# gongaa/Feedback-GNN

Measured on AMD Instinct MI355X. Metric: decoded codewords/sec, [[882,24]] 64-iter BP4 + feedback-GNN, higher is better.
Workload: dtype f32

## Files before the change

### feedback_gnn_amd/_lib.py

```python
import ctypes as C
import os
import subprocess

_HERE = os.path.dirname(os.path.abspath(__file__))
LIB_PATH = os.path.join(_HERE, "lib", "libfgnn_hip.so")
CSRC = os.path.join(_HERE, "csrc")

CN_TYPES = {"boxplus": 0, "boxplus-phi": 1, "minsum": 2}
ROWS_X_LOGIT, ROWS_Z_LOGIT, ROWS_HX_PERP, ROWS_HZ_PERP, ROWS_LX, ROWS_LZ = 0, 1, 2, 3, 4, 5


class FgnnError(RuntimeError):
    pass


def build(force=False, verbose=False):
    cmd = ["make", "-C", CSRC, "-j4"] + (["-B"] if force else [])
    res = subprocess.run(cmd, stdout=subprocess.PIPE, stderr=subprocess.STDOUT, text=True)
    if verbose or res.returncode != 0:
        print(res.stdout)
    if res.returncode != 0:
        raise FgnnError("building libfgnn_hip.so failed")
    return LIB_PATH


KERNEL_SOURCES = {
    "bp4": ("fgnn_bp4.hip", "fgnn_math.h", "fgnn_internal.h", "fgnn_rng.h", "fgnn_cn.h", "Makefile"),
    "gnn": ("fgnn_gnn.hip", "fgnn_math.h", "fgnn_internal.h", "fgnn_pk.h", "fgnn_mlp.h", "Makefile"),
    "gnnbp4": ("fgnn_gnnbp4.hip", "fgnn_math.h", "fgnn_internal.h", "fgnn_pk.h", "fgnn_mlp.h", "Makefile"),
}


def source_fingerprint(kind):
    import hashlib
    h = hashlib.sha256()
    for name in KERNEL_SOURCES[kind]:
        h.update(name.encode() + b"\0")
        with open(os.path.join(CSRC, name), "rb") as f:
            h.update(f.read())
        h.update(b"\0")
    return h.hexdigest()


def library_sha256(path=None):
    import hashlib
    h = hashlib.sha256()
    with open(path or os.environ.get("FGNN_LIB_PATH", LIB_PATH), "rb") as f:
        for blk in iter(lambda: f.read(1 << 20), b""):
            h.update(blk)
    return h.hexdigest()


_SIGNATURES = {
    "fgnn_last_error": (C.c_char_p, []),
    "fgnn_version": (C.c_int, []),
    "fgnn_graph_create": (C.c_int, [C.c_int, C.c_int, C.c_int, C.c_int, C.c_void_p, C.c_void_p, C.c_int, C.c_void_p,
                                    C.c_void_p, C.c_int, C.POINTER(C.c_void_p)]),
    "fgnn_graph_destroy": (None, [C.c_void_p]),
    "fgnn_graph_set_rows": (C.c_int, [C.c_void_p, C.c_int, C.c_int, C.c_int, C.c_void_p, C.c_void_p]),
    "fgnn_graph_set_launch": (C.c_int, [C.c_void_p, C.c_int, C.c_int]),
    "fgnn_graph_set_option": (C.c_int, [C.c_void_p, C.c_int, C.c_int]),
    "fgnn_graph_force_generic": (C.c_int, [C.c_void_p, C.c_int]),
    "fgnn_graph_info": (C.c_int, [C.c_void_p, C.c_void_p]),
    "fgnn_graph_edges": (C.c_int, [C.c_void_p, C.c_int, C.c_void_p, C.c_void_p]),
    "fgnn_profile_enable": (C.c_int, [C.c_void_p, C.c_int]),
    "fgnn_profile_read": (C.c_int, [C.c_void_p, C.c_void_p, C.c_void_p, C.c_void_p, C.c_int, C.c_void_p]),
    "fgnn_bp4_decode": (C.c_int, [C.c_void_p, C.c_int, C.c_int, C.c_float, C.c_void_p, C.c_float, C.c_void_p, C.c_void_p,
                                  C.c_int] + [C.c_void_p] * 10),
    "fgnn_bp4_decode_trace": (C.c_int, [C.c_void_p, C.c_int, C.c_int, C.c_float, C.c_void_p, C.c_float, C.c_void_p, C.c_void_p,
                                        C.c_int] + [C.c_void_p] * 10),
    "fgnn_weights_create": (C.c_int, [C.c_void_p, C.c_int, C.POINTER(C.c_void_p)]),
    "fgnn_weights_destroy": (None, [C.c_void_p]),
    "fgnn_feedback_gnn": (C.c_int, [C.c_void_p] * 7 + [C.c_int, C.c_void_p, C.c_void_p]),
    "fgnn_pauli_noise": (C.c_int, [C.c_uint64, C.c_float, C.c_uint64, C.c_int, C.c_int, C.c_void_p, C.c_void_p, C.c_void_p]),
    "fgnn_pauli_noise_xyz": (C.c_int, [C.c_uint64, C.c_float, C.c_float, C.c_float, C.c_uint64, C.c_int, C.c_int, C.c_void_p, C.c_void_p, C.c_void_p]),
    "fgnn_pauli_noise_wt": (C.c_int, [C.c_uint64, C.c_int, C.c_uint64, C.c_int, C.c_int, C.c_void_p, C.c_void_p, C.c_void_p]),
    "fgnn_pauli_noise_dev": (C.c_int, [C.c_uint64, C.c_float, C.c_void_p, C.c_uint64, C.c_int, C.c_int, C.c_void_p, C.c_void_p, C.c_void_p]),
    "fgnn_syndrome": (C.c_int, [C.c_void_p, C.c_void_p, C.c_void_p, C.c_int, C.c_void_p, C.c_void_p, C.c_void_p]),
    "fgnn_flag_update": (C.c_int, [C.c_void_p] * 5 + [C.c_int, C.c_void_p, C.c_void_p]),
    "fgnn_merge": (C.c_int, [C.c_void_p] * 3 + [C.c_int, C.c_int, C.c_void_p, C.c_void_p, C.c_void_p]),
# ... 82 lines not shown
```

### feedback_gnn_amd/csrc/fgnn_bp4.hip

```cpp

#include "fgnn_internal.h"
#include "fgnn_math.h"
#include "fgnn_cn.h"

#ifndef FGNN_BP4_WAVES
#define FGNN_BP4_WAVES 7
#endif
#ifndef FGNN_HWT_PIN_CLIP_POINTS
#define FGNN_HWT_PIN_CLIP_POINTS 1
#endif
#ifndef FGNN_PHI_STAGE
#define FGNN_PHI_STAGE 1
#endif

namespace {

struct BpArgs {
    int B, num_iter, tpc, cpb, lds_per_cw, lch_off;
    float factor, llr_const;
    const float* llr_ch;
    const uint8_t* synd_x;
    const uint8_t* synd_z;
    const float* msg_init_x;
    const float* msg_init_z;
    float* llr_out;
    uint8_t* x_hat;
    uint8_t* z_hat;
    float* x_logit;
    float* z_logit;
    float* msg_out_x;
    float* msg_out_z;
    const int* index;
    int shortcut;
    int early_exit;
    int sig_off;
    int lreg;
    int hwt;
    uint8_t* flagged;
    int flag_off;
    float* gmem;
    float* trace_x;
    float* trace_z;
    int trace_off;
    float* tape_x;
    float* tape_z;
    int shared_lse;
};

template <bool HWT>
struct Mx {
    static __device__ __forceinline__ float softplus(float t) { return fg_softplus(t); }
    static __device__ __forceinline__ float lse2(float a, float b) { return fg_lse2(a, b); }
    static __device__ __forceinline__ float lse2_corr(float a, float b) { return fg_lse2_corr(a, b); }
    static __device__ __forceinline__ float phi(float x) { return fg_phi(x); }
};
template <>
struct Mx<true> {
    static __device__ __forceinline__ float exp(float x) { return __builtin_amdgcn_exp2f(x * FG_LOG2E); }
    static __device__ __forceinline__ float log(float x) { return __builtin_amdgcn_logf(x) * 0.693147182f; }
    static __device__ __forceinline__ float softplus(float t)
    {
        const float y = exp(FG_CLAMP(t, -87.0f, FG_SOFTPLUS_THRESH));
        const float r = (t < -FG_SOFTPLUS_THRESH) ? ((t < -87.0f) ? 0.0f : y) : log(1.0f + y);
        return (t > FG_SOFTPLUS_THRESH) ? t : r;
    }
    static __device__ __forceinline__ float lse2_corr(float a, float b)
    {
        const float y = exp(-FG_MIN(FG_ABS(a - b), 20.0f));
        return log(1.0f + y);
    }
    static __device__ __forceinline__ float lse2(float a, float b)
    {
        return lse2_corr(a, b) + FG_MAX(a, b);
    }
    static __device__ __forceinline__ float phi(float x)
    {
        const float xc = FG_CLAMP(x, FG_PHI_MIN, FG_PHI_MAX);
        const float y = exp(xc);
        const float sp = (xc > FG_SOFTPLUS_THRESH) ? xc : log(1.0f + y);
        float r = sp - log(y - 1.0f);
#if FGNN_HWT_PIN_CLIP_POINTS
        r = (x >= FG_PHI_MAX) ? 0.0f : r;
        r = (x <= FG_PHI_MIN) ? 16.6355324f : r;
#endif
        return r;
    }
};

template <bool HWT = false>
__device__ __forceinline__ float logit_row_opt(const float* llr, const int* __restrict__ col, int deg, float phi0, bool shortcut)
{
    if (shortcut) {
        unsigned neg = 0;
        bool sat = true;
        for (int j = 0; j < deg; ++j) {
            const float v = llr[col[j]];
            neg ^= (v < 0.0f);
            sat = sat && (FG_ABS(v) >= FG_PHI_MAX);
        }
        if (__all(sat)) return with_sign(phi0, neg);
    }
    return logit_row<Mx<HWT>>(llr, col, deg);
}

template <int N, bool HWT = false>
__device__ __forceinline__ void phi_n(const float (&x)[N], float (&out)[N])
{
    if constexpr (HWT) {
#pragma unroll
        for (int k = 0; k < N; ++k) out[k] = Mx<true>::phi(x[k]);
        return;
    }
    const float* tab = fg_log_tab();
    float xc[N], y[N];
    uint32_t eb1[N], eb2[N], j1[N], j2[N];
#pragma unroll
    for (int k = 0; k < N; ++k) {
        xc[k] = FG_CLAMP(x[k], FG_PHI_MIN, FG_PHI_MAX);
        y[k] = fg_exp(xc[k]);
        const uint32_t w1 = fg_f2u(1.0f + y[k]) - FG_LOG_OFFS;
        const uint32_t w2 = fg_f2u(y[k] - 1.0f) - FG_LOG_OFFS;
        eb1[k] = w1 & 0xff800000u;
        eb2[k] = w2 & 0xff800000u;
        j1[k] = (w1 >> 18) & 31u;
        j2[k] = (w2 >> 18) & 31u;
    }
    __builtin_amdgcn_sched_barrier(0);
    float rc1[N], lc1[N], rc2[N], lc2[N];
#pragma unroll
    for (int k = 0; k < N; ++k) {
        rc1[k] = tab[j1[k]];
        lc1[k] = tab[32 + j1[k]];
        rc2[k] = tab[j2[k]];
        lc2[k] = tab[32 + j2[k]];
    }
    __builtin_amdgcn_sched_barrier(0);
#pragma unroll
    for (int k = 0; k < N; ++k) {
        const float a = fg_u2f(fg_f2u(rc1[k]) - eb1[k]);
        const float r1 = FG_FMA(y[k], a, a - 1.0f);
        float sp = FG_FMA((float)(int32_t)eb1[k], FG_LN2_S23, lc1[k] + fg_log1p_small(r1));
        sp = (xc[k] > FG_SOFTPLUS_THRESH) ? xc[k] : sp;
        const float mm = fg_u2f(fg_f2u(y[k] - 1.0f) - eb2[k]);
        const float r2 = FG_FMA(mm, rc2[k], -1.0f);
        const float lg = FG_FMA((float)(int32_t)eb2[k], FG_LN2_S23, lc2[k] + fg_log1p_small(r2));
        out[k] = sp - lg;
    }
}

template <int DC, bool HWT = false, bool F1 = false>
__device__ __forceinline__ bool cn_phi_regular(float* msg, const int (&sl)[DC], unsigned synd, float factor, float phi0,
                                               bool shortcut)
{
    constexpr int H = (DC % FGNN_PHI_STAGE == 0) ? FGNN_PHI_STAGE : DC / 2;
    static_assert(DC % H == 0, "a phi stage must take a whole fraction of a check");
    float v[DC], aa[DC];
    uint32_t neg = synd << 31;
    bool sat = true;
#pragma unroll
    for (int j = 0; j < DC; ++j) {
        v[j] = slot_ref(msg, sl[j]);
        neg ^= fg_f2u(v[j]);
        sat = sat && (FG_ABS(v[j]) >= FG_PHI_MAX);
    }
    if (shortcut && __all(sat)) {
#pragma unroll
        for (int j = 0; j < DC; ++j) {
            const float o = fg_u2f(fg_f2u(phi0) | ((neg ^ fg_f2u(v[j])) & 0x80000000u));
            slot_ref(msg, sl[j]) = F1 ? o : o * factor;
        }
        return true;
    }
#pragma unroll
    for (int g0 = 0; g0 < DC; g0 += H) {
        float xa[H], oa[H];
#pragma unroll
        for (int j = 0; j < H; ++j) xa[j] = FG_ABS(v[g0 + j]);
        phi_n<H, HWT>(xa, oa);
#pragma unroll
        for (int j = 0; j < H; ++j) aa[g0 + j] = oa[j];
    }
    float T = 0.0f;
#pragma unroll
    for (int j = 0; j < DC; ++j) T = T + aa[j];
#pragma unroll
    for (int g0 = 0; g0 < DC; g0 += H) {
        float xa[H], oa[H];
#pragma unroll
        for (int j = 0; j < H; ++j) xa[j] = T - aa[g0 + j];
        phi_n<H, HWT>(xa, oa);
#pragma unroll
        for (int j = 0; j < H; ++j) {
            const float o = fg_u2f(fg_f2u(oa[j]) | ((neg ^ fg_f2u(v[g0 + j])) & 0x80000000u));
            slot_ref(msg, sl[g0 + j]) = F1 ? o : o * factor;
        }
    }
    return false;
}

template <int DC>
__device__ __forceinline__ void cn_tanh_regular(float* msg, const int (&sl)[DC], unsigned synd, float factor)
{
    float t[DC];
    float P = 1.0f;
#pragma unroll
    for (int j = 0; j < DC; ++j) {
        float tj = fg_tanh(slot_ref(msg, sl[j]) / 2.0f);
        tj = (tj == 0.0f) ? 1e-12f : tj;
        P = (j == 0) ? tj : P * tj;
        t[j] = tj;
    }
    P = P * (synd ? -1.0f : 1.0f);
    const float clipv = 0.99999988f;
#pragma unroll
    for (int j = 0; j < DC; ++j) {
        float q = fg_rcp_unit(t[j]) * P;
        q = (FG_ABS(q) < 1e-7f) ? 0.0f : q;
        q = FG_MIN(FG_MAX(q, -clipv), clipv);
        slot_ref(msg, sl[j]) = (2.0f * fg_atanh(q)) * factor;
    }
}

template <bool HWT = false>
__device__ __forceinline__ bool cn_phi_generic(float* msg, const int* __restrict__ slot, int deg, unsigned synd, float factor,
                                               float phi0, bool shortcut)
{
    if (shortcut) {
        unsigned neg = synd;
        bool sat = true;
        for (int j = 0; j < deg; ++j) {
            const float v = msg[slot[j]];
            neg ^= (v < 0.0f);
            sat = sat && (FG_ABS(v) >= FG_PHI_MAX);
        }
        if (__all(sat)) {
            for (int j = 0; j < deg; ++j) {
                const int s = slot[j];
                msg[s] = with_sign(phi0, neg ^ (unsigned)(msg[s] < 0.0f)) * factor;
            }
            return true;
        }
    }
    cn_update<FGNN_CN_BOXPLUS_PHI, Mx<HWT>>(msg, slot, deg, synd, factor);
    return false;
}

__device__ __forceinline__ float softplus_saturated(float t)
{
    const float y = fg_exp(FG_MIN(FG_MAX(t, -87.0f), 0.0f));
    return (t > 0.0f) ? t : ((t < -87.0f) ? 0.0f : y);
}

template <int CN_TYPE, int DVX, int DVZ, int DC, bool OPT, bool HWT = false, int NQ = 0, bool TRACE = false, bool GMEM = false, int LSE = 2>
__global__ void __launch_bounds__(1024) __attribute__((amdgpu_waves_per_eu(NQ > 0 ? FGNN_BP4_WAVES - 1 : FGNN_BP4_WAVES)))
bp4_kernel(GraphDev g, BpArgs a)
{
    static_assert(!(HWT && OPT), "the hardware-transcendental variant is the fixed dataflow only: the exact shortcuts are proofs about fgnn_math.h");
    static_assert(!GMEM || (DVX == 0 && !OPT && !HWT && NQ == 0 && !TRACE), "the global-memory variant is the plain runtime-degree kernel");
    using MX = Mx<HWT>;
    FG_LOG_TAB_SETUP();
    constexpr bool REGULAR = DVX > 0;
    constexpr bool LREG = NQ > 0;
    constexpr int NQA = LREG ? NQ : 1;
    const bool opt_shortcut = OPT && a.shortcut != 0;
    const bool opt_exit = OPT && a.early_exit != 0;
    const bool shl = LSE == 2 ? a.shared_lse != 0 : LSE == 1;
    extern __shared__ float lds[];
    const int cwl = threadIdx.x / a.tpc;
    const int lane = threadIdx.x - cwl * a.tpc;
    const int slot_b = blockIdx.x * a.cpb + cwl;
    const bool active = slot_b < a.B;
    const int b = (active && a.index) ? a.index[slot_b] : slot_b;
    float* msg;
    if constexpr (GMEM) msg = a.gmem + (size_t)slot_b * a.lds_per_cw;
    else msg = lds + (size_t)cwl * a.lds_per_cw;
    float* Lch = msg + a.lch_off;
    const int n = g.n;

    constexpr bool CLOSED_OK = REGULAR && CN_TYPE == FGNN_CN_BOXPLUS_PHI && !LREG && !TRACE;
    const bool zero_start = REGULAR && !TRACE && !a.msg_init_x && !a.msg_init_z && a.num_iter > 0;
    const bool first_closed = CLOSED_OK && zero_start && !a.llr_ch;
    const bool first_peeled = zero_start && a.llr_ch != nullptr;
    const bool fill = !first_closed && !first_peeled;
    if (active) {
        if (fill) {
            for (int e = lane; e < g.E_x; e += a.tpc) msg[e] = a.msg_init_x ? a.msg_init_x[(size_t)b * g.E_x + e] : 0.0f;
            for (int e = lane; e < g.E_z; e += a.tpc)
                msg[g.E_x + e] = a.msg_init_z ? a.msg_init_z[(size_t)b * g.E_z + e] : 0.0f;
        }
        if (a.llr_ch && !LREG)
            for (int i = lane; i < 3 * n; i += a.tpc) Lch[i] = a.llr_ch[(size_t)b * 3 * n + i];
    }
    float lreg[3][NQA];
    if constexpr (LREG) {
#pragma unroll
        for (int i = 0; i < NQ; ++i) {
            const int v = lane + i * a.tpc;
            const bool in = active && v < n;
#pragma unroll
            for (int c = 0; c < 3; ++c) lreg[c][i] = in ? a.llr_ch[(size_t)b * 3 * n + c * n + v] : 0.0f;
        }
    }
    if (fill || (a.llr_ch && !LREG)) __syncthreads();

    const uint8_t* sx = a.synd_x + (size_t)b * g.m_x;
    const uint8_t* sz = a.synd_z + (size_t)b * g.m_z;
    const int lane_c = lane + (a.tpc >> 1) < a.tpc ? lane + (a.tpc >> 1) : lane - a.tpc + (a.tpc >> 1);

    const float phi0 = MX::phi(0.0f);
    (void)phi0;
    unsigned* sigw = reinterpret_cast<unsigned*>(msg + a.sig_off);
    int* flags = reinterpret_cast<int*>(sigw + n);
    bool a1 = false, a2 = false;
    if (opt_exit) {
        for (int v = lane; v < n; v += a.tpc) sigw[v] = fill ? 0xffffffffu : 0u;
        if (lane < 4) flags[lane] = 0;
        __syncthreads();
    }
    int it_begin = 0;
    if constexpr (CLOSED_OK) {
        if (first_closed) {
            const float L = a.llr_const;
            const float Y = (0.0f + 0.0f) + L, X = 0.0f + L, Z = 0.0f + L;
            const float nu_x = MX::softplus(-X) - MX::lse2(-(Z - 0.0f), -(Y - 0.0f));
            const float nu_z = MX::softplus(-Z) - MX::lse2(-(X - 0.0f), -(Y - 0.0f));
            if (active)
                for (int c = lane_c; c < g.m; c += a.tpc) {
                    const unsigned synd = (c < g.m_x ? sx[c] : sz[c - g.m_x]) & 1u;
                    const uint4 pk = reinterpret_cast<const uint4*>(g.cslot16)[c];
                    const unsigned w[4] = {pk.x, pk.y, pk.z, pk.w};
                    const float nu = c < g.m_x ? nu_x : nu_z;
                    const unsigned ng = nu < 0.0f;
                    unsigned neg = synd;
                    const float aa = MX::phi(FG_ABS(nu));
                    float T = 0.0f;
#pragma unroll
                    for (int j = 0; j < DC; ++j) {
                        neg ^= ng;
                        T = T + aa;
                    }
                    const float val = with_sign(MX::phi(T - aa), neg ^ ng) * a.factor;
#pragma unroll
                    for (int j = 0; j < DC; ++j) slot_ref(msg, (int)((w[j >> 1] >> ((j & 1) * 16)) & 0xffffu)) = val;
                }
            if (opt_exit) a1 = FG_ABS(nu_x) >= FG_PHI_MAX && FG_ABS(nu_z) >= FG_PHI_MAX;
            it_begin = 1;
            __syncthreads();
        }
    }
    const bool cn_one = a.cpb == 1, cn_f1 = a.factor == 1.0f;
    unsigned synd_bits = 0;
    if (active) {
        int i = 0;
        for (int c = lane_c; c < g.m && i < 32; c += a.tpc, ++i) synd_bits |= ((c < g.m_x ? sx[c] : sz[c - g.m_x]) & 1u) << i;
    }
    const bool synd_in_reg = (g.m + a.tpc - 1) / a.tpc <= 32;
    auto trace_step = [&](const int k) __attribute__((always_inline)) {
        float* tlx = msg + a.trace_off;
        float* tlz = tlx + n;
        if (active && a.tape_x) {
            float* px = a.tape_x + ((size_t)k * a.B + b) * g.E_x;
            float* pz = a.tape_z + ((size_t)k * a.B + b) * g.E_z;
            for (int e = lane; e < g.E_x; e += a.tpc) px[e] = msg[e];
            for (int e = lane; e < g.E_z; e += a.tpc) pz[e] = msg[g.E_x + e];
        }
        if (active)
            for (int v = lane; v < n; v += a.tpc) {
                const int x0 = g.vptr_x[v], x1 = g.vptr_x[v + 1], z0 = g.vptr_z[v], z1 = g.vptr_z[v + 1];
                float Sz = 0.0f, Sx = 0.0f;
                for (int e = z0; e < z1; ++e) Sz = Sz + msg[e];
                for (int e = x0; e < x1; ++e) Sx = Sx + msg[e];
                const float lx = a.llr_ch ? Lch[v] : a.llr_const, ly = a.llr_ch ? Lch[n + v] : a.llr_const,
                            lz = a.llr_ch ? Lch[2 * n + v] : a.llr_const;
                const float Y = (Sz + Sx) + ly;
                const float X = Sz + lx;
                const float Z = Sx + lz;
                tlz[v] = MX::softplus(-X) - MX::lse2(-Z, -Y);
                tlx[v] = MX::softplus(-Z) - MX::lse2(-X, -Y);
            }
        __syncthreads();
        if (active) {
            float* tx = a.trace_x + ((size_t)k * a.B + b) * g.rows[0];
            for (int r = lane; r < g.rows[0]; r += a.tpc) {
                const int p0 = g.rptr[0][r];
                tx[r] = logit_row<Mx<HWT>>(tlx, g.rcol[0] + p0, g.rptr[0][r + 1] - p0);
            }
            float* tz = a.trace_z + ((size_t)k * a.B + b) * g.rows[1];
            for (int r = lane; r < g.rows[1]; r += a.tpc) {
                const int p0 = g.rptr[1][r];
                tz[r] = logit_row<Mx<HWT>>(tlz, g.rcol[1] + p0, g.rptr[1][r + 1] - p0);
            }
        }
    };
    if constexpr (TRACE) trace_step(0);
    if constexpr (REGULAR && !TRACE) {
        if (first_peeled && active) {
            auto vn_first = [&](const int v, const float lx, const float ly, const float lz) __attribute__((always_inline)) {
                const float Y = (0.0f + 0.0f) + ly;
                const float X = 0.0f + lx;
                const float Z = 0.0f + lz;
                const float numx = MX::softplus(-X);
                const float numz = MX::softplus(-Z);
                const float Ze = Z - 0.0f, Xe = X - 0.0f, Ye = Y - 0.0f;
                float ox, oz;
                if (shl) {
                    ox = numx - (MX::lse2_corr(-Z, -Y) + FG_MAX(-Ze, -Ye));
                    oz = numz - (MX::lse2_corr(-X, -Y) + FG_MAX(-Xe, -Ye));
                } else {
                    ox = numx - MX::lse2(-Ze, -Ye);
                    oz = numz - MX::lse2(-Xe, -Ye);
                }
                float* px = msg + v * DVX;
                float* pz = msg + g.E_x + v * DVZ;
#pragma unroll
                for (int k = 0; k < DVX; ++k) px[k] = ox;
#pragma unroll
                for (int k = 0; k < DVZ; ++k) pz[k] = oz;
            };
            if constexpr (LREG) {
#pragma unroll
                for (int i = 0; i < NQ; ++i) {
                    const int v = lane + i * a.tpc;
                    if (v < n) vn_first(v, lreg[0][i], lreg[1][i], lreg[2][i]);
                }
            } else {
                for (int v = lane; v < n; v += a.tpc) vn_first(v, Lch[v], Lch[n + v], Lch[2 * n + v]);
            }
        }
    }
    for (int it = it_begin; it < a.num_iter; ++it) {
        bool changed = false, cn_slow = false;
        auto vn_body = [&](const int v, const float lx, const float ly, const float lz) __attribute__((always_inline)) {
                if constexpr (REGULAR) {
                    float* px = msg + v * DVX;
                    float* pz = msg + g.E_x + v * DVZ;
                    float mx[DVX], mz[DVZ];
                    float Sz = 0.0f, Sx = 0.0f;
#pragma unroll
                    for (int k = 0; k < DVZ; ++k) { mz[k] = pz[k]; Sz = Sz + mz[k]; }
#pragma unroll
                    for (int k = 0; k < DVX; ++k) { mx[k] = px[k]; Sx = Sx + mx[k]; }
                    if (opt_exit) {
                        unsigned sig = 0;
#pragma unroll
                        for (int k = 0; k < DVX; ++k) sig |= sign_bit(mx[k]) << k;
#pragma unroll
                        for (int k = 0; k < DVZ; ++k) sig |= sign_bit(mz[k]) << (DVX + k);
                        if (sigw[v] != sig) {
                            changed = true;
                            sigw[v] = sig;
                        }
                    }
                    const float Y = (Sz + Sx) + ly;
                    const float X = Sz + lx;
                    const float Z = Sx + lz;
                    bool sat = opt_shortcut && FG_ABS(X) > FG_SOFTPLUS_THRESH && FG_ABS(Z) > FG_SOFTPLUS_THRESH;
                    if (shl) {
                        sat = sat && FG_ABS((-Z) - (-Y)) >= 20.0f && FG_ABS((-X) - (-Y)) >= 20.0f;
                    } else {
#pragma unroll
                        for (int k = 0; k < DVX; ++k) sat = sat && (FG_ABS((Z - mx[k]) - (Y - mx[k])) >= 20.0f);
#pragma unroll
                        for (int k = 0; k < DVZ; ++k) sat = sat && (FG_ABS((X - mz[k]) - (Y - mz[k])) >= 20.0f);
                    }
                    if (opt_shortcut && __all(sat)) {
                        const float numx = softplus_saturated(-X);
                        const float numz = softplus_saturated(-Z);
#pragma unroll
                        for (int k = 0; k < DVX; ++k) {
                            const float Ze = Z - mx[k], Ye = Y - mx[k];
                            px[k] = numx - (0.0f + FG_MAX(-Ze, -Ye));
                        }
#pragma unroll
                        for (int k = 0; k < DVZ; ++k) {
                            const float Xe = X - mz[k], Ye = Y - mz[k];
                            pz[k] = numz - (0.0f + FG_MAX(-Xe, -Ye));
                        }
                        return;
                    }
// ... 46 lines not shown
                            sig |= sign_bit(mm) << ((x1 - x0) + (e - z0));
                        }
                        if (opt_exit && sigw[v] != sig) {
                            changed = true;
                            sigw[v] = sig;
                        }
                        if (__all(sat)) {
                            const float nx = softplus_saturated(-X), nz = softplus_saturated(-Z);
                            for (int e = x0; e < x1; ++e) {
                                const float mm = msg[e];
                                const float Ze = Z - mm, Ye = Y - mm;
                                msg[e] = nx - (0.0f + FG_MAX(-Ze, -Ye));
                            }
                            for (int e = z0; e < z1; ++e) {
                                const float mm = msg[e];
                                const float Xe = X - mm, Ye = Y - mm;
                                msg[e] = nz - (0.0f + FG_MAX(-Xe, -Ye));
                            }
                            return;
                        }
                    }
                    const float numx = MX::softplus(-X);
                    const float numz = MX::softplus(-Z);
                    if (shl) {
                        const float cx = MX::lse2_corr(-Z, -Y), cz = MX::lse2_corr(-X, -Y);
                        for (int e = x0; e < x1; ++e) {
                            float m = msg[e];
                            float Ze = Z - m, Ye = Y - m;
                            msg[e] = numx - (cx + FG_MAX(-Ze, -Ye));
                        }
                        for (int e = z0; e < z1; ++e) {
                            float m = msg[e];
                            float Xe = X - m, Ye = Y - m;
                            msg[e] = numz - (cz + FG_MAX(-Xe, -Ye));
                        }
                        return;
                    }
                    for (int e = x0; e < x1; ++e) {
                        float m = msg[e];
                        float Ze = Z - m, Ye = Y - m;
                        msg[e] = numx - MX::lse2(-Ze, -Ye);
                    }
                    for (int e = z0; e < z1; ++e) {
                        float m = msg[e];
                        float Xe = X - m, Ye = Y - m;
                        msg[e] = numz - MX::lse2(-Xe, -Ye);
                    }
                }
            };
        if (active && !(first_peeled && it == 0)) {
            if constexpr (LREG) {
#pragma unroll
                for (int i = 0; i < NQ; ++i) {
                    const int v = lane + i * a.tpc;
                    if (v < n) vn_body(v, lreg[0][i], lreg[1][i], lreg[2][i]);
                }
            } else {
                for (int v = lane; v < n; v += a.tpc) {
                    if (a.llr_ch) vn_body(v, Lch[v], Lch[n + v], Lch[2 * n + v]);
                    else vn_body(v, a.llr_const, a.llr_const, a.llr_const);
                }
            }
        }
        if (opt_exit && changed) flags[2 * (it & 1)] = 1;
        __syncthreads();
        if (opt_exit && lane == 0) {
            flags[2 * ((it + 1) & 1)] = 0;
            flags[2 * ((it + 1) & 1) + 1] = 0;
        }
        if (active) {
            int ci = 0;
            for (int c = lane_c; c < g.m; c += a.tpc, ++ci) {
                const unsigned synd = synd_in_reg ? (synd_bits >> ci) & 1u : (c < g.m_x ? sx[c] : sz[c - g.m_x]) & 1u;
                if constexpr (REGULAR) {
                    const uint4 pk = reinterpret_cast<const uint4*>(g.cslot16)[c];
                    const unsigned w[4] = {pk.x, pk.y, pk.z, pk.w};
                    int sl[DC];
#pragma unroll
                    for (int j = 0; j < DC; ++j) sl[j] = (int)((w[j >> 1] >> ((j & 1) * 16)) & 0xffffu);
                    if constexpr (CN_TYPE == FGNN_CN_BOXPLUS_PHI) {
                        bool fast;
                        if (cn_one && cn_f1) fast = cn_phi_regular<DC, HWT, true>(lds, sl, synd, 1.0f, phi0, opt_shortcut);
                        else if (cn_one) fast = cn_phi_regular<DC, HWT, false>(lds, sl, synd, a.factor, phi0, opt_shortcut);
                        else fast = cn_phi_regular<DC, HWT, false>(msg, sl, synd, a.factor, phi0, opt_shortcut);
                        cn_slow = !fast || cn_slow;
                    } else if constexpr (CN_TYPE == FGNN_CN_MINSUM) {
                        cn_minsum_regular<DC>(msg, sl, DC, synd, a.factor);
                    } else {
                        cn_tanh_regular<DC>(msg, sl, synd, a.factor);
                    }
                } else {
                    const int c0 = g.cptr[c], deg = g.cptr[c + 1] - c0;
                    if constexpr (CN_TYPE == FGNN_CN_BOXPLUS_PHI)
                        cn_slow = !cn_phi_generic<HWT>(msg, g.cslot + c0, deg, synd, a.factor, phi0, opt_shortcut) || cn_slow;
                    else cn_update<CN_TYPE, Mx<HWT>>(msg, g.cslot + c0, deg, synd, a.factor);
                }
            }
        }
        if (opt_exit && cn_slow) flags[2 * (it & 1) + 1] = 1;
        __syncthreads();
        if (opt_exit) {
            const bool stable = a1 && a2 && flags[2 * (it & 1)] == 0;
            a2 = a1;
            a1 = flags[2 * (it & 1) + 1] == 0;
            if (stable) break;
        }
        if constexpr (TRACE) trace_step(it + 1);
    }

    if (active) {
        if (a.msg_out_x)
            for (int e = lane; e < g.E_x; e += a.tpc) a.msg_out_x[(size_t)b * g.E_x + e] = msg[e];
        if (a.msg_out_z)
            for (int e = lane; e < g.E_z; e += a.tpc) a.msg_out_z[(size_t)b * g.E_z + e] = msg[g.E_x + e];
    }
    auto total_body = [&](const int v, const float lx, const float ly, const float lz) __attribute__((always_inline)) {
            const int x0 = g.vptr_x[v], x1 = g.vptr_x[v + 1], z0 = g.vptr_z[v], z1 = g.vptr_z[v + 1];
            float Sz = 0.0f, Sx = 0.0f;
            for (int e = z0; e < z1; ++e) Sz = Sz + msg[e];
            for (int e = x0; e < x1; ++e) Sx = Sx + msg[e];
            const float Y = (Sz + Sx) + ly;
            const float X = Sz + lx;
            const float Z = Sx + lz;
            float* o = a.llr_out + (size_t)b * 3 * n;
            o[v] = X;
            o[n + v] = Y;
            o[2 * n + v] = Z;
            int d = 0;
            float best = 0.0f;
            if (X < best) { best = X; d = 1; }
            if (Z < best) { best = Z; d = 2; }
            if (Y < best) { best = Y; d = 3; }
            a.x_hat[(size_t)b * n + v] = (uint8_t)(d & 1);
            a.z_hat[(size_t)b * n + v] = (uint8_t)(d >> 1);
    };
    if (active) {
        if constexpr (LREG) {
#pragma unroll
            for (int i = 0; i < NQ; ++i) {
                const int v = lane + i * a.tpc;
                if (v < n) total_body(v, lreg[0][i], lreg[1][i], lreg[2][i]);
            }
        } else {
            for (int v = lane; v < n; v += a.tpc) {
                if (a.llr_ch) total_body(v, Lch[v], Lch[n + v], Lch[2 * n + v]);
                else total_body(v, a.llr_const, a.llr_const, a.llr_const);
            }
        }
    }
    if (a.flagged) {
        uint8_t* dec = reinterpret_cast<uint8_t*>(msg + a.flag_off);
        unsigned* fword = reinterpret_cast<unsigned*>(dec + ((n + 3) & ~3));
        __syncthreads();
        if (active)
            for (int v = lane; v < n; v += a.tpc) {
                dec[v] = (uint8_t)(a.x_hat[(size_t)b * n + v] | (a.z_hat[(size_t)b * n + v] << 1));
            }
        if (lane == 0) *fword = 0u;
        __syncthreads();
        unsigned mine = 0;
        if (active)
            for (int c = lane; c < g.m; c += a.tpc) {
                const int sh = c < g.m_x ? 1 : 0;
                unsigned par = (c < g.m_x ? sx[c] : sz[c - g.m_x]) & 1u;
                for (int e = g.cptr[c]; e < g.cptr[c + 1]; ++e) par ^= (dec[g.cvn[e]] >> sh) & 1u;
                mine |= par;
            }
        if (mine) atomicOr(fword, 1u);
        __syncthreads();
        if (active && lane == 0) a.flagged[b] = (uint8_t)(*fword != 0u);
    }
    if (!a.x_logit && !a.z_logit) return;
    __syncthreads();
    float* llx = msg;
    float* llz = msg + n;
    if (active)
        for (int v = lane; v < n; v += a.tpc) {
            const float* o = a.llr_out + (size_t)b * 3 * n;
            const float X = o[v], Y = o[n + v], Z = o[2 * n + v];
            const bool sat = opt_shortcut && FG_ABS(X) > FG_SOFTPLUS_THRESH && FG_ABS(Z) > FG_SOFTPLUS_THRESH &&
                             FG_ABS((-Z) - (-Y)) >= 20.0f && FG_ABS((-X) - (-Y)) >= 20.0f;
            if (opt_shortcut && __all(sat)) {
                llz[v] = softplus_saturated(-X) - (0.0f + FG_MAX(-Z, -Y));
                llx[v] = softplus_saturated(-Z) - (0.0f + FG_MAX(-X, -Y));
                continue;
            }
            llz[v] = MX::softplus(-X) - MX::lse2(-Z, -Y);
            llx[v] = MX::softplus(-Z) - MX::lse2(-X, -Y);
        }
    __syncthreads();
    if (active) {
        if (a.x_logit)
            for (int r = lane; r < g.rows[0]; r += a.tpc) {
                const int p0 = g.rptr[0][r];
                a.x_logit[(size_t)b * g.rows[0] + r] = logit_row_opt<HWT>(llx, g.rcol[0] + p0, g.rptr[0][r + 1] - p0, phi0, opt_shortcut);
            }
        if (a.z_logit)
            for (int r = lane; r < g.rows[1]; r += a.tpc) {
                const int p0 = g.rptr[1][r];
                a.z_logit[(size_t)b * g.rows[1] + r] = logit_row_opt<HWT>(llz, g.rcol[1] + p0, g.rptr[1][r + 1] - p0, phi0, opt_shortcut);
            }
    }
}

using Bp4Kernel = void (*)(GraphDev, BpArgs);

template <int NQ, bool OPT, int LSE>
constexpr Bp4Kernel bp4_lse_kernel = bp4_kernel<FGNN_CN_BOXPLUS_PHI, 3, 3, 6, OPT, false, NQ, false, false, LSE>;
constexpr Bp4Kernel bp4_lse_kernels[3][2][2] = {
    {{bp4_lse_kernel<0, false, 0>, bp4_lse_kernel<0, false, 1>}, {bp4_lse_kernel<0, true, 0>, bp4_lse_kernel<0, true, 1>}},
    {{bp4_lse_kernel<4, false, 0>, bp4_lse_kernel<4, false, 1>}, {bp4_lse_kernel<4, true, 0>, bp4_lse_kernel<4, true, 1>}},
    {{bp4_lse_kernel<5, false, 0>, bp4_lse_kernel<5, false, 1>}, {bp4_lse_kernel<5, true, 0>, bp4_lse_kernel<5, true, 1>}}};

template <int CN_TYPE, int DVX, int DVZ, int DC>
int launch_bp4_k(const fgnn_graph* g, const BpArgs& a, const LaunchGeom& L, size_t lds_bytes, hipStream_t st)
{
    Bp4Kernel kern = a.shortcut ? bp4_kernel<CN_TYPE, DVX, DVZ, DC, true> : bp4_kernel<CN_TYPE, DVX, DVZ, DC, false>;
    if constexpr ((DVX == 3 && DVZ == 3 && DC == 6) || DVX == 0) {
        if (a.trace_x) kern = bp4_kernel<CN_TYPE, DVX, DVZ, DC, false, false, 0, true>;
    }
    if constexpr (CN_TYPE == FGNN_CN_BOXPLUS_PHI) {
        if (a.hwt) kern = bp4_kernel<CN_TYPE, DVX, DVZ, DC, false, true>;
        if constexpr (DVX == 3 && DVZ == 3 && DC == 6) {
            if (!a.trace_x && !a.hwt) kern = bp4_lse_kernels[a.lreg ? a.lreg - 3 : 0][a.shortcut][a.shared_lse];
        }
    }
    return fgnn_launch(kern, dim3(L.blocks), dim3(L.threads), lds_bytes, st, g->d, a);
}

struct Bp4Plan {
    size_t lds_bytes;
    bool gmem;
    size_t ws_bytes;
};

template <int CN_TYPE>
int launch_bp4(const fgnn_graph* g, const BpArgs& a, const LaunchGeom& L, const Bp4Plan& p, hipStream_t st)
{
    if (p.gmem)
        return fgnn_launch(bp4_kernel<CN_TYPE, 0, 0, 0, false, false, 0, false, true>, dim3(L.blocks), dim3(L.threads), 0, st, g->d, a);
    const GraphDev& d = g->d;
    if (d.cslot16 && !g->force_generic) {
        if (d.dvx == 3 && d.dvz == 3 && d.dc == 6) return launch_bp4_k<CN_TYPE, 3, 3, 6>(g, a, L, p.lds_bytes, st);
        if (d.dvx == 4 && d.dvz == 4 && d.dc == 8 && !a.trace_x) return launch_bp4_k<CN_TYPE, 4, 4, 8>(g, a, L, p.lds_bytes, st);
    }
    return launch_bp4_k<CN_TYPE, 0, 0, 0>(g, a, L, p.lds_bytes, st);
}

Bp4Plan plan_bp4(const fgnn_graph* g, int cn_type, const LaunchGeom& L, BpArgs& a, bool gmem = false)
{
    const GraphDev& d = g->d;
    const int n = d.n;
    const bool trace = a.trace_x != nullptr, phi = cn_type == FGNN_CN_BOXPLUS_PHI;
    auto round4 = [](int floats) { return (floats + 3) & ~3; };
    a.shared_lse = g->bp4_shared_lse ? 1 : 0;
    a.hwt = (g->hw_transcendentals && phi && !trace && !gmem) ? 1 : 0;
    a.shortcut = (g->shortcut && !a.hwt && !trace && !gmem) ? 1 : 0;
    a.lch_off = d.E > 2 * n ? d.E : 2 * n;
    const int per_thread = (n + L.tpc - 1) / L.tpc;
    const bool r336 = d.cslot16 && !g->force_generic && d.dvx == 3 && d.dvz == 3 && d.dc == 6;
    a.lreg = (a.llr_ch && !trace && !a.hwt && !gmem && phi && L.cpb == 1 && r336 && per_thread <= 5) ? (per_thread <= 4 ? 4 : 5) : 0;
    int per = a.lch_off + ((a.llr_ch && !a.lreg) ? 3 * n : 0);
    a.trace_off = 0;
    if (trace) {
        a.trace_off = per;
        per += 2 * n;
    }
    if (!gmem) per = round4(per);
    a.sig_off = per;
    int tail = 0;
    a.early_exit = (a.shortcut && g->early_exit && d.max_vdeg <= 32 && phi && L.cpb == 1 && a.num_iter > 2) ? 1 : 0;
    if (a.early_exit) {
        if (((size_t)per * L.cpb + n + 4) * sizeof(float) <= FGNN_LDS_BUDGET) tail += n + 4;
        else a.early_exit = 0;
    }
    a.flag_off = 0;
    if (a.flagged) {
        const int need = round4(n) / 4 + 1;
        if (a.lch_off >= 2 * n + need) {
            a.flag_off = 2 * n;
        } else {
            a.flag_off = per + tail;
            tail += need;
        }
    }
    if (gmem) {
        a.lds_per_cw = round4(per + tail);
        return {0, true, (size_t)L.blocks * (size_t)a.lds_per_cw * sizeof(float)};
    }
    a.lds_per_cw = per;
    const size_t lds_bytes = ((size_t)per * L.cpb + tail) * sizeof(float);
    if (lds_bytes > FGNN_LDS_BUDGET) return plan_bp4(g, cn_type, L, a, true);
    return {lds_bytes, false, 0};
}

}

static int bp4_decode_core(const fgnn_graph* g, int cn_type, int num_iter, float normalization_factor, const float* llr_ch,
                           float llr_const, const uint8_t* synd_x, const uint8_t* synd_z, int B, const float* msg_init_x,
                           const float* msg_init_z, float* llr_out, uint8_t* x_hat, uint8_t* z_hat, float* x_logit,
                           float* z_logit, float* msg_out_x, float* msg_out_z, const int* index, uint8_t* flagged,
                           float* trace_x, float* trace_z, float* tape_x, float* tape_z, void* stream)
{
    if (!g) return fgnn_fail(FGNN_ERR_ARG, "graph is NULL");
    if (B < 0 || num_iter < 0) return fgnn_fail(FGNN_ERR_ARG, "B and num_iter must be >= 0");
    if (cn_type < 0 || cn_type > 2) return fgnn_fail(FGNN_ERR_ARG, "Unknown node type.");
    if ((x_logit && !g->d.rptr[0]) || (z_logit && !g->d.rptr[1]))
        return fgnn_fail(FGNN_ERR_STATE, "logit row sets not installed (fgnn_graph_set_rows)");
    if (B == 0) return FGNN_OK;
    if (!synd_x || !synd_z || !llr_out || !x_hat || !z_hat) return fgnn_fail(FGNN_ERR_ARG, "required buffer is NULL");
    FGNN_DEVICE_GUARD(g->device);
    const LaunchGeom L = fgnn_geom(g, B);
    if (flagged && L.cpb != 1) return fgnn_fail(FGNN_ERR_STATE, "the fused flag test needs one codeword per workgroup");
    BpArgs a;
// ... 92 lines not shown
```

Baseline: 951,500.

## Add compile-time trip-count BP4 kernel and range-restricted lse2 log

```diff
diff --git a/feedback_gnn_amd/_lib.py b/feedback_gnn_amd/_lib.py
--- a/feedback_gnn_amd/_lib.py
+++ b/feedback_gnn_amd/_lib.py
@@ -25,7 +25,7 @@
 
 
 KERNEL_SOURCES = {
-    "bp4": ("fgnn_bp4.hip", "fgnn_math.h", "fgnn_internal.h", "fgnn_rng.h", "fgnn_cn.h", "Makefile"),
+    "bp4": ("fgnn_bp4.hip", "fgnn_math.h", "fgnn_math_ranged.h", "fgnn_internal.h", "fgnn_rng.h", "fgnn_cn.h", "Makefile"),
     "gnn": ("fgnn_gnn.hip", "fgnn_math.h", "fgnn_internal.h", "fgnn_pk.h", "fgnn_mlp.h", "Makefile"),
     "gnnbp4": ("fgnn_gnnbp4.hip", "fgnn_math.h", "fgnn_internal.h", "fgnn_pk.h", "fgnn_mlp.h", "Makefile"),
 }
diff --git a/feedback_gnn_amd/csrc/fgnn_bp4.hip b/feedback_gnn_amd/csrc/fgnn_bp4.hip
--- a/feedback_gnn_amd/csrc/fgnn_bp4.hip
+++ b/feedback_gnn_amd/csrc/fgnn_bp4.hip
@@ -1,6 +1,9 @@
+
+#include <type_traits>
 
 #include "fgnn_internal.h"
 #include "fgnn_math.h"
+#include "fgnn_math_ranged.h"
 #include "fgnn_cn.h"
 
 #ifndef FGNN_BP4_WAVES
@@ -44,14 +47,15 @@
     int trace_off;
     float* tape_x;
     float* tape_z;
+    int nt;
     int shared_lse;
 };
 
 template <bool HWT>
 struct Mx {
     static __device__ __forceinline__ float softplus(float t) { return fg_softplus(t); }
-    static __device__ __forceinline__ float lse2(float a, float b) { return fg_lse2(a, b); }
-    static __device__ __forceinline__ float lse2_corr(float a, float b) { return fg_lse2_corr(a, b); }
+    static __device__ __forceinline__ float lse2(float a, float b) { return fg_lse2_ranged(a, b); }
+    static __device__ __forceinline__ float lse2_corr(float a, float b) { return fg_lse2_corr_ranged(a, b); }
     static __device__ __forceinline__ float phi(float x) { return fg_phi(x); }
 };
 template <>
@@ -149,13 +153,13 @@
 }
 
 template <int DC, bool HWT = false, bool F1 = false>
-__device__ __forceinline__ bool cn_phi_regular(float* msg, const int (&sl)[DC], unsigned synd, float factor, float phi0,
+__device__ __forceinline__ bool cn_phi_regular(float* msg, const int (&sl)[DC], uint32_t neg0, float factor, float phi0,
                                                bool shortcut)
 {
     constexpr int H = (DC % FGNN_PHI_STAGE == 0) ? FGNN_PHI_STAGE : DC / 2;
     static_assert(DC % H == 0, "a phi stage must take a whole fraction of a check");
     float v[DC], aa[DC];
-    uint32_t neg = synd << 31;
+    uint32_t neg = neg0;
     bool sat = true;
 #pragma unroll
     for (int j = 0; j < DC; ++j) {
@@ -251,7 +255,8 @@
     return (t > 0.0f) ? t : ((t < -87.0f) ? 0.0f : y);
 }
 
-template <int CN_TYPE, int DVX, int DVZ, int DC, bool OPT, bool HWT = false, int NQ = 0, bool TRACE = false, bool GMEM = false, int LSE = 2>
+template <int CN_TYPE, int DVX, int DVZ, int DC, bool OPT, bool HWT = false, int NQ = 0, bool TRACE = false, bool GMEM = false, int LSE = 2,
+          int NT = 0>
 __global__ void __launch_bounds__(1024) __attribute__((amdgpu_waves_per_eu(NQ > 0 ? FGNN_BP4_WAVES - 1 : FGNN_BP4_WAVES)))
 bp4_kernel(GraphDev g, BpArgs a)
 {
@@ -262,17 +267,21 @@
     constexpr bool REGULAR = DVX > 0;
     constexpr bool LREG = NQ > 0;
     constexpr int NQA = LREG ? NQ : 1;
+    static_assert(NT == 0 || (DVX > 0 && CN_TYPE == FGNN_CN_BOXPLUS_PHI && !LREG && !TRACE && !GMEM), "compile-time trips: the regular phi kernel");
+    constexpr int CT = LREG ? NQ : NT;
+    const int tpc = NT > 0 ? 256 : a.tpc;
     const bool opt_shortcut = OPT && a.shortcut != 0;
     const bool opt_exit = OPT && a.early_exit != 0;
     const bool shl = LSE == 2 ? a.shared_lse != 0 : LSE == 1;
     extern __shared__ float lds[];
-    const int cwl = threadIdx.x / a.tpc;
-    const int lane = threadIdx.x - cwl * a.tpc;
-    const int slot_b = blockIdx.x * a.cpb + cwl;
+    const int cwl = NT > 0 ? 0 : threadIdx.x / tpc;
+    const int lane = threadIdx.x - cwl * tpc;
+    const int slot_b = NT > 0 ? blockIdx.x : blockIdx.x * a.cpb + cwl;
     const bool active = slot_b < a.B;
     const int b = (active && a.index) ? a.index[slot_b] : slot_b;
     float* msg;
     if constexpr (GMEM) msg = a.gmem + (size_t)slot_b * a.lds_per_cw;
+    else if constexpr (NT > 0) msg = lds;
     else msg = lds + (size_t)cwl * a.lds_per_cw;
     float* Lch = msg + a.lch_off;
     const int n = g.n;
@@ -284,18 +293,18 @@
     const bool fill = !first_closed && !first_peeled;
     if (active) {
         if (fill) {
-            for (int e = lane; e < g.E_x; e += a.tpc) msg[e] = a.msg_init_x ? a.msg_init_x[(size_t)b * g.E_x + e] : 0.0f;
-            for (int e = lane; e < g.E_z; e += a.tpc)
+            for (int e = lane; e < g.E_x; e += tpc) msg[e] = a.msg_init_x ? a.msg_init_x[(size_t)b * g.E_x + e] : 0.0f;
+            for (int e = lane; e < g.E_z; e += tpc)
                 msg[g.E_x + e] = a.msg_init_z ? a.msg_init_z[(size_t)b * g.E_z + e] : 0.0f;
         }
         if (a.llr_ch && !LREG)
-            for (int i = lane; i < 3 * n; i += a.tpc) Lch[i] = a.llr_ch[(size_t)b * 3 * n + i];
+            for (int i = lane; i < 3 * n; i += tpc) Lch[i] = a.llr_ch[(size_t)b * 3 * n + i];
     }
     float lreg[3][NQA];
     if constexpr (LREG) {
 #pragma unroll
         for (int i = 0; i < NQ; ++i) {
-            const int v = lane + i * a.tpc;
+            const int v = lane + i * tpc;
             const bool in = active && v < n;
 #pragma unroll
             for (int c = 0; c < 3; ++c) lreg[c][i] = in ? a.llr_ch[(size_t)b * 3 * n + c * n + v] : 0.0f;
@@ -305,7 +314,7 @@
 
     const uint8_t* sx = a.synd_x + (size_t)b * g.m_x;
     const uint8_t* sz = a.synd_z + (size_t)b * g.m_z;
-    const int lane_c = lane + (a.tpc >> 1) < a.tpc ? lane + (a.tpc >> 1) : lane - a.tpc + (a.tpc >> 1);
+    const int lane_c = lane + (tpc >> 1) < tpc ? lane + (tpc >> 1) : lane - tpc + (tpc >> 1);
 
     const float phi0 = MX::phi(0.0f);
     (void)phi0;
@@ -313,7 +322,7 @@
     int* flags = reinterpret_cast<int*>(sigw + n);
     bool a1 = false, a2 = false;
     if (opt_exit) {
-        for (int v = lane; v < n; v += a.tpc) sigw[v] = fill ? 0xffffffffu : 0u;
+        for (int v = lane; v < n; v += tpc) sigw[v] = fill ? 0xffffffffu : 0u;
         if (lane < 4) flags[lane] = 0;
         __syncthreads();
     }
@@ -325,7 +334,7 @@
             const float nu_x = MX::softplus(-X) - MX::lse2(-(Z - 0.0f), -(Y - 0.0f));
             const float nu_z = MX::softplus(-Z) - MX::lse2(-(X - 0.0f), -(Y - 0.0f));
             if (active)
-                for (int c = lane_c; c < g.m; c += a.tpc) {
+                for (int c = lane_c; c < g.m; c += tpc) {
                     const unsigned synd = (c < g.m_x ? sx[c] : sz[c - g.m_x]) & 1u;
                     const uint4 pk = reinterpret_cast<const uint4*>(g.cslot16)[c];
                     const unsigned w[4] = {pk.x, pk.y, pk.z, pk.w};
@@ -352,20 +361,21 @@
     unsigned synd_bits = 0;
     if (active) {
         int i = 0;
-        for (int c = lane_c; c < g.m && i < 32; c += a.tpc, ++i) synd_bits |= ((c < g.m_x ? sx[c] : sz[c - g.m_x]) & 1u) << i;
-    }
-    const bool synd_in_reg = (g.m + a.tpc - 1) / a.tpc <= 32;
+        for (int c = lane_c; c < g.m && i < 32; c += tpc, ++i) synd_bits |= ((c < g.m_x ? sx[c] : sz[c - g.m_x]) & 1u) << i;
+    }
+    const bool synd_in_reg = (g.m + tpc - 1) / tpc <= 32;
+    unsigned row_off = 16u * (unsigned)lane_c;
     auto trace_step = [&](const int k) __attribute__((always_inline)) {
         float* tlx = msg + a.trace_off;
         float* tlz = tlx + n;
         if (active && a.tape_x) {
             float* px = a.tape_x + ((size_t)k * a.B + b) * g.E_x;
             float* pz = a.tape_z + ((size_t)k * a.B + b) * g.E_z;
-            for (int e = lane; e < g.E_x; e += a.tpc) px[e] = msg[e];
-            for (int e = lane; e < g.E_z; e += a.tpc) pz[e] = msg[g.E_x + e];
+            for (int e = lane; e < g.E_x; e += tpc) px[e] = msg[e];
+            for (int e = lane; e < g.E_z; e += tpc) pz[e] = msg[g.E_x + e];
         }
         if (active)
-            for (int v = lane; v < n; v += a.tpc) {
+            for (int v = lane; v < n; v += tpc) {
                 const int x0 = g.vptr_x[v], x1 = g.vptr_x[v + 1], z0 = g.vptr_z[v], z1 = g.vptr_z[v + 1];
                 float Sz = 0.0f, Sx = 0.0f;
                 for (int e = z0; e < z1; ++e) Sz = Sz + msg[e];
@@ -381,12 +391,12 @@
         __syncthreads();
         if (active) {
             float* tx = a.trace_x + ((size_t)k * a.B + b) * g.rows[0];
-            for (int r = lane; r < g.rows[0]; r += a.tpc) {
+            for (int r = lane; r < g.rows[0]; r += tpc) {
                 const int p0 = g.rptr[0][r];
                 tx[r] = logit_row<Mx<HWT>>(tlx, g.rcol[0] + p0, g.rptr[0][r + 1] - p0);
             }
             float* tz = a.trace_z + ((size_t)k * a.B + b) * g.rows[1];
-            for (int r = lane; r < g.rows[1]; r += a.tpc) {
+            for (int r = lane; r < g.rows[1]; r += tpc) {
                 const int p0 = g.rptr[1][r];
                 tz[r] = logit_row<Mx<HWT>>(tlz, g.rcol[1] + p0, g.rptr[1][r + 1] - p0);
             }
@@ -420,11 +430,11 @@
             if constexpr (LREG) {
 #pragma unroll
                 for (int i = 0; i < NQ; ++i) {
-                    const int v = lane + i * a.tpc;
+                    const int v = lane + i * tpc;
                     if (v < n) vn_first(v, lreg[0][i], lreg[1][i], lreg[2][i]);
                 }
             } else {
-                for (int v = lane; v < n; v += a.tpc) vn_first(v, Lch[v], Lch[n + v], Lch[2 * n + v]);
+                for (int v = lane; v < n; v += tpc) vn_first(v, Lch[v], Lch[n + v], Lch[2 * n + v]);
             }
         }
     }
@@ -577,11 +587,17 @@
             if constexpr (LREG) {
 #pragma unroll
                 for (int i = 0; i < NQ; ++i) {
-                    const int v = lane + i * a.tpc;
+                    const int v = lane + i * tpc;
                     if (v < n) vn_body(v, lreg[0][i], lreg[1][i], lreg[2][i]);
                 }
+            } else if constexpr (NT > 0) {
+#pragma unroll
+                for (int i = 0; i < NT; ++i) {
+                    const int v = lane + i * 256;
+                    if (i + 1 < NT || v < n) vn_body(v, a.llr_const, a.llr_const, a.llr_const);
+                }
             } else {
-                for (int v = lane; v < n; v += a.tpc) {
+                for (int v = lane; v < n; v += tpc) {
                     if (a.llr_ch) vn_body(v, Lch[v], Lch[n + v], Lch[2 * n + v]);
                     else vn_body(v, a.llr_const, a.llr_const, a.llr_const);
                 }
@@ -593,9 +609,35 @@
             flags[2 * ((it + 1) & 1)] = 0;
             flags[2 * ((it + 1) & 1) + 1] = 0;
         }
-        if (active) {
+        if constexpr (REGULAR && CT > 0 && CN_TYPE == FGNN_CN_BOXPLUS_PHI) {
+            auto cn_trips = [&](auto f1) __attribute__((always_inline)) {
+                constexpr bool F1 = decltype(f1)::value;
+                const char* rows = reinterpret_cast<const char*>(g.cslot16);
+#pragma unroll
+                for (int i = 0; i < CT; ++i) {
+                    const bool in = (!LREG && i + 1 < CT) || lane_c + i * tpc < g.m;
+                    if (in) {
+                        const char* base = rows + (size_t)i * (size_t)(16u * (unsigned)tpc);
+                        asm volatile("" : "+v"(row_off));
+                        if constexpr (NT > 0) asm volatile("" : "+s"(base));
+                        typedef unsigned Row __attribute__((ext_vector_type(4)));
+                        const Row pk = *(const __attribute__((address_space(1))) Row*)(base + row_off);
+                        const unsigned w[4] = {pk.x, pk.y, pk.z, pk.w};
+                        int sl[DC];
+#pragma unroll
+                        for (int j = 0; j < DC; ++j) sl[j] = (int)((w[j >> 1] >> ((j & 1) * 16)) & 0xffffu);
+                        const bool fast = cn_phi_regular<DC, HWT, F1>(lds, sl, synd_bits << (31 - i), F1 ? 1.0f : a.factor, phi0, opt_shortcut);
+                        cn_slow = !fast || cn_slow;
+                    }
+                }
+            };
+            if (active) {
+                if (cn_f1) cn_trips(std::true_type{});
+                else cn_trips(std::false_type{});
+            }
+        } else if (active) {
             int ci = 0;
-            for (int c = lane_c; c < g.m; c += a.tpc, ++ci) {
+            for (int c = lane_c; c < g.m; c += tpc, ++ci) {
                 const unsigned synd = synd_in_reg ? (synd_bits >> ci) & 1u : (c < g.m_x ? sx[c] : sz[c - g.m_x]) & 1u;
                 if constexpr (REGULAR) {
                     const uint4 pk = reinterpret_cast<const uint4*>(g.cslot16)[c];
@@ -605,9 +647,9 @@
                     for (int j = 0; j < DC; ++j) sl[j] = (int)((w[j >> 1] >> ((j & 1) * 16)) & 0xffffu);
                     if constexpr (CN_TYPE == FGNN_CN_BOXPLUS_PHI) {
                         bool fast;
-                        if (cn_one && cn_f1) fast = cn_phi_regular<DC, HWT, true>(lds, sl, synd, 1.0f, phi0, opt_shortcut);
-                        else if (cn_one) fast = cn_phi_regular<DC, HWT, false>(lds, sl, synd, a.factor, phi0, opt_shortcut);
-                        else fast = cn_phi_regular<DC, HWT, false>(msg, sl, synd, a.factor, phi0, opt_shortcut);
+                        if (cn_one && cn_f1) fast = cn_phi_regular<DC, HWT, true>(lds, sl, synd << 31, 1.0f, phi0, opt_shortcut);
+                        else if (cn_one) fast = cn_phi_regular<DC, HWT, false>(lds, sl, synd << 31, a.factor, phi0, opt_shortcut);
+                        else fast = cn_phi_regular<DC, HWT, false>(msg, sl, synd << 31, a.factor, phi0, opt_shortcut);
                         cn_slow = !fast || cn_slow;
                     } else if constexpr (CN_TYPE == FGNN_CN_MINSUM) {
                         cn_minsum_regular<DC>(msg, sl, DC, synd, a.factor);
@@ -635,9 +677,9 @@
 
     if (active) {
         if (a.msg_out_x)
-            for (int e = lane; e < g.E_x; e += a.tpc) a.msg_out_x[(size_t)b * g.E_x + e] = msg[e];
+            for (int e = lane; e < g.E_x; e += tpc) a.msg_out_x[(size_t)b * g.E_x + e] = msg[e];
         if (a.msg_out_z)
-            for (int e = lane; e < g.E_z; e += a.tpc) a.msg_out_z[(size_t)b * g.E_z + e] = msg[g.E_x + e];
+            for (int e = lane; e < g.E_z; e += tpc) a.msg_out_z[(size_t)b * g.E_z + e] = msg[g.E_x + e];
     }
     auto total_body = [&](const int v, const float lx, const float ly, const float lz) __attribute__((always_inline)) {
             const int x0 = g.vptr_x[v], x1 = g.vptr_x[v + 1], z0 = g.vptr_z[v], z1 = g.vptr_z[v + 1];
@@ -663,11 +705,11 @@
         if constexpr (LREG) {
 #pragma unroll
             for (int i = 0; i < NQ; ++i) {
-                const int v = lane + i * a.tpc;
+                const int v = lane + i * tpc;
                 if (v < n) total_body(v, lreg[0][i], lreg[1][i], lreg[2][i]);
             }
         } else {
-            for (int v = lane; v < n; v += a.tpc) {
+            for (int v = lane; v < n; v += tpc) {
                 if (a.llr_ch) total_body(v, Lch[v], Lch[n + v], Lch[2 * n + v]);
                 else total_body(v, a.llr_const, a.llr_const, a.llr_const);
             }
@@ -678,14 +720,14 @@
         unsigned* fword = reinterpret_cast<unsigned*>(dec + ((n + 3) & ~3));
         __syncthreads();
         if (active)
-            for (int v = lane; v < n; v += a.tpc) {
+            for (int v = lane; v < n; v += tpc) {
                 dec[v] = (uint8_t)(a.x_hat[(size_t)b * n + v] | (a.z_hat[(size_t)b * n + v] << 1));
             }
         if (lane == 0) *fword = 0u;
         __syncthreads();
         unsigned mine = 0;
         if (active)
-            for (int c = lane; c < g.m; c += a.tpc) {
+            for (int c = lane; c < g.m; c += tpc) {
                 const int sh = c < g.m_x ? 1 : 0;
                 unsigned par = (c < g.m_x ? sx[c] : sz[c - g.m_x]) & 1u;
                 for (int e = g.cptr[c]; e < g.cptr[c + 1]; ++e) par ^= (dec[g.cvn[e]] >> sh) & 1u;
@@ -700,7 +742,7 @@
     float* llx = msg;
     float* llz = msg + n;
     if (active)
-        for (int v = lane; v < n; v += a.tpc) {
+        for (int v = lane; v < n; v += tpc) {
             const float* o = a.llr_out + (size_t)b * 3 * n;
             const float X = o[v], Y = o[n + v], Z = o[2 * n + v];
             const bool sat = opt_shortcut && FG_ABS(X) > FG_SOFTPLUS_THRESH && FG_ABS(Z) > FG_SOFTPLUS_THRESH &&
@@ -716,12 +758,12 @@
     __syncthreads();
     if (active) {
         if (a.x_logit)
-            for (int r = lane; r < g.rows[0]; r += a.tpc) {
+            for (int r = lane; r < g.rows[0]; r += tpc) {
                 const int p0 = g.rptr[0][r];
                 a.x_logit[(size_t)b * g.rows[0] + r] = logit_row_opt<HWT>(llx, g.rcol[0] + p0, g.rptr[0][r + 1] - p0, phi0, opt_shortcut);
             }
         if (a.z_logit)
-            for (int r = lane; r < g.rows[1]; r += a.tpc) {
+            for (int r = lane; r < g.rows[1]; r += tpc) {
                 const int p0 = g.rptr[1][r];
                 a.z_logit[(size_t)b * g.rows[1] + r] = logit_row_opt<HWT>(llz, g.rcol[1] + p0, g.rptr[1][r + 1] - p0, phi0, opt_shortcut);
             }
@@ -730,13 +772,17 @@
 
 using Bp4Kernel = void (*)(GraphDev, BpArgs);
 
-template <int NQ, bool OPT, int LSE>
-constexpr Bp4Kernel bp4_lse_kernel = bp4_kernel<FGNN_CN_BOXPLUS_PHI, 3, 3, 6, OPT, false, NQ, false, false, LSE>;
+template <int NQ, bool OPT, int LSE, int NT = 0>
+constexpr Bp4Kernel bp4_lse_kernel = bp4_kernel<FGNN_CN_BOXPLUS_PHI, 3, 3, 6, OPT, false, NQ, false, false, LSE, NT>;
 constexpr Bp4Kernel bp4_lse_kernels[3][2][2] = {
     {{bp4_lse_kernel<0, false, 0>, bp4_lse_kernel<0, false, 1>}, {bp4_lse_kernel<0, true, 0>, bp4_lse_kernel<0, true, 1>}},
     {{bp4_lse_kernel<4, false, 0>, bp4_lse_kernel<4, false, 1>}, {bp4_lse_kernel<4, true, 0>, bp4_lse_kernel<4, true, 1>}},
     {{bp4_lse_kernel<5, false, 0>, bp4_lse_kernel<5, false, 1>}, {bp4_lse_kernel<5, true, 0>, bp4_lse_kernel<5, true, 1>}}};
 
+constexpr Bp4Kernel bp4_nt_kernels[2][2][2] = {
+    {{bp4_lse_kernel<0, false, 0, 4>, bp4_lse_kernel<0, false, 1, 4>}, {bp4_lse_kernel<0, true, 0, 4>, bp4_lse_kernel<0, true, 1, 4>}},
+    {{bp4_lse_kernel<0, false, 0, 5>, bp4_lse_kernel<0, false, 1, 5>}, {bp4_lse_kernel<0, true, 0, 5>, bp4_lse_kernel<0, true, 1, 5>}}};
+
 template <int CN_TYPE, int DVX, int DVZ, int DC>
 int launch_bp4_k(const fgnn_graph* g, const BpArgs& a, const LaunchGeom& L, size_t lds_bytes, hipStream_t st)
 {
@@ -748,6 +794,7 @@
         if (a.hwt) kern = bp4_kernel<CN_TYPE, DVX, DVZ, DC, false, true>;
         if constexpr (DVX == 3 && DVZ == 3 && DC == 6) {
             if (!a.trace_x && !a.hwt) kern = bp4_lse_kernels[a.lreg ? a.lreg - 3 : 0][a.shortcut][a.shared_lse];
+            if (!a.trace_x && !a.hwt && a.nt) kern = bp4_nt_kernels[a.nt - 4][a.shortcut][a.shared_lse];
         }
     }
     return fgnn_launch(kern, dim3(L.blocks), dim3(L.threads), lds_bytes, st, g->d, a);
@@ -782,9 +829,12 @@
     a.hwt = (g->hw_transcendentals && phi && !trace && !gmem) ? 1 : 0;
     a.shortcut = (g->shortcut && !a.hwt && !trace && !gmem) ? 1 : 0;
     a.lch_off = d.E > 2 * n ? d.E : 2 * n;
-    const int per_thread = (n + L.tpc - 1) / L.tpc;
+    const int per_thread = (n + L.tpc - 1) / L.tpc, per_thread_c = (d.m + L.tpc - 1) / L.tpc;
+    const int trips = per_thread > per_thread_c ? per_thread : per_thread_c;
     const bool r336 = d.cslot16 && !g->force_generic && d.dvx == 3 && d.dvz == 3 && d.dc == 6;
-    a.lreg = (a.llr_ch && !trace && !a.hwt && !gmem && phi && L.cpb == 1 && r336 && per_thread <= 5) ? (per_thread <= 4 ? 4 : 5) : 0;
+    const bool fixed_trips = !trace && !a.hwt && !gmem && phi && L.cpb == 1 && r336;
+    a.lreg = (a.llr_ch && fixed_trips && trips <= 5) ? (trips <= 4 ? 4 : 5) : 0;
+    a.nt = (!a.llr_ch && fixed_trips && L.tpc == 256 && per_thread == per_thread_c && (trips == 4 || trips == 5)) ? trips : 0;
     int per = a.lch_off + ((a.llr_ch && !a.lreg) ? 3 * n : 0);
     a.trace_off = 0;
     if (trace) {
diff --git a/feedback_gnn_amd/csrc/fgnn_math_ranged.h b/feedback_gnn_amd/csrc/fgnn_math_ranged.h
--- /dev/null
+++ b/feedback_gnn_amd/csrc/fgnn_math_ranged.h
@@ -0,0 +1,33 @@
+#ifndef FGNN_MATH_RANGED_H
+#define FGNN_MATH_RANGED_H
+
+#include "fgnn_math.h"
+
+#define FG_LN2_S126 0x1.62e43p+125f
+
+FG_FN float fg_log_1to2(float x)
+{
+    const float* tab = fg_log_tab();
+    const uint32_t b = fg_f2u(x);
+    const uint32_t w = b - FG_LOG_OFFS;
+    const uint32_t eb = w & 0xff800000u;
+    const float mm = fg_u2f(b - eb);
+    const uint32_t j = (w >> 18) & 31u;
+    const float rc = tab[j], lc = tab[32 + j];
+    const float r = FG_FMA(mm, rc, -1.0f);
+    return FG_FMA(fg_u2f(eb), FG_LN2_S126, lc + fg_log1p_small(r));
+}
+
+FG_FN float fg_lse2_corr_ranged(float a, float b)
+{
+    float d = FG_ABS(a - b);
+    float y = fg_exp(-FG_MIN(d, 20.0f));
+    return fg_log_1to2(1.0f + y);
+}
+FG_FN float fg_lse2_ranged(float a, float b)
+{
+    float m = FG_MAX(a, b);
+    return fg_lse2_corr_ranged(a, b) + m;
+}
+
+#endif
```

New measurement: 976,000 (median of 6 runs). +2.6%, better.
